# NTV-UIT/MARLLB

Hardware: NVIDIA B200
Metric: agent-steps/sec (higher is better)
Workload: dtype f32

## Files before the change

### marllb_b200/csrc/mlb_features.cuh

```cuda
#pragma once
#include "mlb_common.cuh"

namespace mlb {

#define MLB_WP_MARGIN 5e-5f

template <int EPL, int SIZE, int STRIDE>
__device__ __forceinline__ void bitonic_stage(float (&k)[EPL], float (&p)[EPL], int lane) {
    if constexpr (STRIDE >= EPL) {
        constexpr int LSTRIDE = STRIDE / EPL;
        const bool keep_min = (((lane * EPL) & SIZE) == 0) == ((lane & LSTRIDE) == 0);
#pragma unroll
        for (int r = 0; r < EPL; r++) {
            const float ok = __shfl_xor_sync(MLB_FULL, k[r], LSTRIDE);
            const float op = __shfl_xor_sync(MLB_FULL, p[r], LSTRIDE);
            const float nk = keep_min ? fminf(k[r], ok) : fmaxf(k[r], ok);
            p[r] = (nk != k[r]) ? op : p[r];
            k[r] = nk;
        }
    } else {
#pragma unroll
        for (int r = 0; r < EPL; r++) {
            if ((r & STRIDE) == 0) {
                const int r2 = r | STRIDE;
// ... 181 lines not shown
    __syncwarp();
    bool ambiguous;
    int idx = weighted_index_scan_f64(vw, n, tmax, decay, &ambiguous);
    if (ambiguous) idx = weighted_index_f64(vw, n, now, decay);
    return idx;
}

__device__ __forceinline__ float fast_rcp(float x) {
    float y;
    asm("rcp.approx.ftz.f32 %0, %1;" : "=f"(y) : "f"(x));
    return y;
}
__device__ __forceinline__ float fast_sqrt(float x) {
    float y;
    asm("sqrt.approx.ftz.f32 %0, %1;" : "=f"(y) : "f"(x));
    return y;
}

template <int EPL, bool FULL>
__device__ __forceinline__ void features_ranked(const float (&v)[EPL], const float (&t)[EPL],
                                                const int (&rk)[EPL], int n_, float now, double decay,
                                                float log2_decay, const WarpScratch& sc, float (&out)[5]) {
    const int lane = lane_id();
    const int s0 = lane * EPL;
    const int n = FULL ? 32 * EPL : n_;
    float s = 0.f, tmax = -MLB_INF;
#pragma unroll
    for (int r = 0; r < EPL; r++) {
        const bool valid = FULL || s0 + r < n;
        s += valid ? v[r] : 0.f;
        tmax = valid ? fmaxf(tmax, t[r]) : tmax;
    }
    const float nf = (float)n;
    const float mean = warp_sum(s) / nf;
    tmax = f32_from_orderable(__reduce_max_sync(MLB_FULL, f32_orderable(tmax)));
    float s2 = 0.f, svw = 0.f;
#pragma unroll
    for (int r = 0; r < EPL; r++) {
        const bool valid = FULL || s0 + r < n;
        const float d = v[r] - mean;
        s2 += valid ? d * d : 0.f;
        const float w = valid ? fast_exp2(log2_decay * (tmax - t[r])) : 0.f;
        svw += valid ? v[r] * w : 0.f;
        const int pos = valid ? rk[r] : s0 + r;
        sc.vw[pos] = make_float2(v[r], w);
    }
    const float sd = fast_sqrt(warp_sum(s2) / nf);
    svw = warp_sum(svw);
    __syncwarp();
    float cum[EPL];
    float sw = 0.f;
#pragma unroll
    for (int r = 0; r < EPL; r += 2) {
        if constexpr (EPL == 1) {
            sw += sc.vw[s0].y;
            cum[0] = sw;
        } else {
            const float4 q = *reinterpret_cast<const float4*>(sc.vw + s0 + r);
            sw += q.y;
            cum[r] = sw;
            sw += q.w;
            cum[r + 1] = sw;
        }
    }
    const float incl = warp_scan_incl(sw, lane);
    const float W = __shfl_sync(MLB_FULL, incl, 31);
    const float mean_decay = svw * fast_rcp(W);
    const float rel = 0.9f * W - (incl - sw);
    int below = 0;
    float dmin = MLB_INF;
#pragma unroll
    for (int r = 0; r < EPL; r++) {
        const bool valid = FULL || s0 + r < n;
        below += (valid && cum[r] < rel) ? 1 : 0;
        dmin = valid ? fminf(dmin, fabsf(cum[r] - rel)) : dmin;
    }
    int idx = __reduce_add_sync(MLB_FULL, below);
    const uint32_t dmin_bits = __reduce_min_sync(MLB_FULL, __float_as_uint(dmin));
    if (__uint_as_float(dmin_bits) < MLB_WP_MARGIN * W) {
        SlotVals<EPL> tv;
        uint32_t packed = 0;
#pragma unroll
        for (int r = 0; r < EPL; r++) {
            tv.x[r] = t[r];
            packed |= (uint32_t)(rk[r] & 255) << (8 * r);
        }
        idx = weighted_index_exact<EPL>(tv, packed, n, tmax, now, decay, sc.vw);
    }
    idx = idx > n - 1 ? n - 1 : idx;
    const float vidx = (float)(n - 1) * (90.0f / 100.0f);
    const float fl = floorf(vidx);
    int lo = (int)fl, hi = lo + 1;
    if (vidx >= (float)(n - 1)) { lo = n - 1; hi = n - 1; }
    hi = hi > n - 1 ? n - 1 : hi;
    const float gamma = vidx - fl;
    const float a = sc.vw[lo].x, b = sc.vw[hi].x;
    const float p90_decay = sc.vw[idx].x;
    const float diff = __fsub_rn(b, a);
    float p90 = __fadd_rn(a, __fmul_rn(diff, gamma));
    if (gamma >= 0.5f) p90 = __fsub_rn(b, __fmul_rn(diff, __fsub_rn(1.0f, gamma)));
    __syncwarp();
    out[0] = mean;
    out[1] = p90;
    out[2] = sd;
    out[3] = mean_decay;
    out[4] = p90_decay;
}

template <int EPL>
__device__ __forceinline__ void features_sorted_epl(const float* __restrict__ vals, const float* __restrict__ tss,
                                                    uint8_t* __restrict__ ranks, int n, float now, double decay,
                                                    float log2_decay, const WarpScratch& sc, float (&out)[5]) {
    const int lane = lane_id();
    float v[EPL], t[EPL];
    int rk[EPL];
    load_slots<EPL>(vals, lane, v);
    load_slots<EPL>(tss, lane, t);
    ranks_full_sort<EPL>(v, n, rk, sc);
    if (ranks) store_ranks<EPL>(ranks, lane, rk);
    if (n == 32 * EPL)
        features_ranked<EPL, true>(v, t, rk, n, now, decay, log2_decay, sc, out);
    else
        features_ranked<EPL, false>(v, t, rk, n, now, decay, log2_decay, sc, out);
}

__device__ __forceinline__ float half_sum(float v) {
#pragma unroll
    for (int o = 8; o > 0; o >>= 1) v += __shfl_xor_sync(MLB_FULL, v, o, 16);
    return v;
}
__device__ __forceinline__ uint32_t half_reduce_add_u16(uint32_t x, int half) {
    const uint32_t both = __reduce_add_sync(MLB_FULL, half ? (x << 16) : x);
    return half ? (both >> 16) : (both & 0xffffu);
}
__device__ __forceinline__ uint32_t half_reduce_max(uint32_t x, int half) {
    const uint32_t m0 = __reduce_max_sync(MLB_FULL, half ? 0u : x);
    const uint32_t m1 = __reduce_max_sync(MLB_FULL, half ? x : 0u);
    return half ? m1 : m0;
}
__device__ __forceinline__ uint32_t half_reduce_min(uint32_t x, int half) {
    const uint32_t m0 = __reduce_min_sync(MLB_FULL, half ? 0xffffffffu : x);
    const uint32_t m1 = __reduce_min_sync(MLB_FULL, half ? x : 0xffffffffu);
    return half ? m1 : m0;
}

template <typename T>
__device__ __forceinline__ T pick8(const T (&x)[8], int sub) {
    const T a = (sub & 1) ? x[1] : x[0], b = (sub & 1) ? x[3] : x[2];
    const T c = (sub & 1) ? x[5] : x[4], d = (sub & 1) ? x[7] : x[6];
    const T lo = (sub & 2) ? b : a, hi = (sub & 2) ? d : c;
    return (sub & 4) ? hi : lo;
}

__device__ __forceinline__ void rank_replace_one_h16(const float (&v)[8], uint32_t (&rkp)[2], int c, int hl,
                                                     int half) {
    const int sub = c & 7, lc = c >> 3;
    const float x = __shfl_sync(MLB_FULL, pick8(v, sub), lc, 16) + 0.0f;
    const uint32_t wsel = (sub & 4) ? rkp[1] : rkp[0];
    const uint32_t r_old = (__shfl_sync(MLB_FULL, wsel, lc, 16) >> (8 * (sub & 3))) & 255u;
    const uint32_t xb = __float_as_uint(x);
    const float xup = __uint_as_float((xb >> 31) ? xb - 1u : xb + 1u);
    const int dl = c - hl * 8;
    uint32_t bef0 = 0, bef1 = 0;
#pragma unroll
    for (int r = 0; r < 4; r++) {
        bef0 |= v[r] < (r == dl ? x : xup) ? (1u << (8 * r)) : 0u;
        bef1 |= v[r + 4] < (r + 4 == dl ? x : xup) ? (1u << (8 * r)) : 0u;
    }
    const uint32_t r_new = half_reduce_add_u16((uint32_t)(__popc(bef0) + __popc(bef1)), half);
    const uint32_t rep = (r_old + 1u) * 0x01010101u;
    rkp[0] = rkp[0] - ((((rkp[0] | 0x80808080u) - rep) >> 7) & 0x01010101u) + (bef0 ^ 0x01010101u);
    rkp[1] = rkp[1] - ((((rkp[1] | 0x80808080u) - rep) >> 7) & 0x01010101u) + (bef1 ^ 0x01010101u);
    if (hl == lc) {
        const int sh = 8 * (sub & 3);
        if (sub & 4) rkp[1] = (rkp[1] & ~(255u << sh)) | (r_new << sh);
        else rkp[0] = (rkp[0] & ~(255u << sh)) | (r_new << sh);
    }
}

__device__ __forceinline__ bool features_full_h16(const float (&v)[8], const float (&t)[8], const uint32_t (&rkp)[2],
                                                  float log2_decay, float2* vw, int hl, int half,
                                                  float (&out)[5]) {
    const float s = ((v[0] + v[1]) + (v[2] + v[3])) + ((v[4] + v[5]) + (v[6] + v[7]));
    const float tm = fmaxf(fmaxf(fmaxf(t[0], t[1]), fmaxf(t[2], t[3])), fmaxf(fmaxf(t[4], t[5]), fmaxf(t[6], t[7])));
    const float mean = half_sum(s) * (1.0f / 128.0f);
    const float tmax = f32_from_orderable(half_reduce_max(f32_orderable(tm), half));
    float s2 = 0.f, svw = 0.f;
#pragma unroll
    for (int r = 0; r < 8; r++) {
        const float dv = v[r] - mean;
        s2 += dv * dv;
        const float w = fast_exp2(log2_decay * (tmax - t[r]));
        svw += v[r] * w;
        const uint32_t pos = (rkp[r >> 2] >> (8 * (r & 3))) & 255u;
        vw[((pos & 7u) << 4) | (pos >> 3)] = make_float2(v[r], w);
    }
    const float sd = fast_sqrt(half_sum(s2) * (1.0f / 128.0f));
    svw = half_sum(svw);
    __syncwarp();
    float cum[8];
    float sw = 0.f;
#pragma unroll
    for (int r = 0; r < 8; r++) {
        sw += vw[r * 16 + hl].y;
        cum[r] = sw;
    }
    float incl = sw;
#pragma unroll
    for (int o = 1; o < 16; o <<= 1) {
        const float y = __shfl_up_sync(MLB_FULL, incl, o, 16);
        if (hl >= o) incl += y;
    }
    const float W = __shfl_sync(MLB_FULL, incl, 15, 16);
    const float mean_decay = svw * fast_rcp(W);
    const float rel = 0.9f * W - (incl - sw);
    int below = 0;
    float dmin = MLB_INF;
#pragma unroll
    for (int r = 0; r < 8; r++) {
        below += cum[r] < rel ? 1 : 0;
        dmin = fminf(dmin, fabsf(cum[r] - rel));
    }
    int idx = (int)half_reduce_add_u16((uint32_t)below, half);
    const uint32_t dmin_bits = half_reduce_min(__float_as_uint(dmin), half);
    const bool ok = !(__uint_as_float(dmin_bits) < MLB_WP_MARGIN * W);
    idx = idx > 127 ? 127 : idx;
    const float vidx = 127.0f * (90.0f / 100.0f);
    const float fl = floorf(vidx);
    const int lo = (int)fl, hi = lo + 1;
    const float gamma = vidx - fl;
    const float a = vw[((lo & 7) << 4) | (lo >> 3)].x, b = vw[((hi & 7) << 4) | (hi >> 3)].x;
    const float p90_decay = vw[((idx & 7) << 4) | (idx >> 3)].x;
    const float diff = __fsub_rn(b, a);
    float p90 = __fadd_rn(a, __fmul_rn(diff, gamma));
    if (gamma >= 0.5f) p90 = __fsub_rn(b, __fmul_rn(diff, __fsub_rn(1.0f, gamma)));
    __syncwarp();
    out[0] = mean;
    out[1] = p90;
    out[2] = sd;
    out[3] = mean_decay;
    out[4] = p90_decay;
    return ok;
}

__device__ __forceinline__ void rank_update_h16(const float (&v)[8], uint32_t (&rkp)[2], uint32_t list, int nchg,
                                                int n_old, int hl, int half) {
    const int s0 = hl * 8;
    uint32_t pm0 = 0, pm1 = 0;
#pragma unroll
    for (int r = 0; r < 4; r++) {
        pm0 |= (s0 + r < n_old) ? (1u << (8 * r)) : 0u;
        pm1 |= (s0 + 4 + r < n_old) ? (1u << (8 * r)) : 0u;
    }
#pragma unroll 1
    for (int k = 0; k < 3; k++) {
        const int c = (list >> (7 * k)) & 127;
        const bool rem = k < nchg && c < n_old;
        if (!__any_sync(MLB_FULL, rem)) continue;
        const int sub = c & 7, lc = c >> 3;
        const uint32_t wsel = (sub & 4) ? rkp[1] : rkp[0];
        const uint32_t r_old = (__shfl_sync(MLB_FULL, wsel, lc, 16) >> (8 * (sub & 3))) & 255u;
        const uint32_t rep = ((r_old & 127u) + 1u) * 0x01010101u;
        const uint32_t g0 = ((((rkp[0] | 0x80808080u) - rep) >> 7) & pm0);
        const uint32_t g1 = ((((rkp[1] | 0x80808080u) - rep) >> 7) & pm1);
        if (rem) {
            rkp[0] -= g0;
            rkp[1] -= g1;
            if (hl == lc) {
                if (sub & 4) pm1 &= ~(1u << (8 * (sub & 3))); else pm0 &= ~(1u << (8 * (sub & 3)));
            }
        }
    }
#pragma unroll 1
    for (int k = 0; k < 3; k++) {
        const bool ins = k < nchg;
        if (!__any_sync(MLB_FULL, ins)) break;
        const int c = (list >> (7 * k)) & 127;
        const int sub = c & 7, lc = c >> 3;
        const float x = __shfl_sync(MLB_FULL, pick8(v, sub), lc, 16) + 0.0f;
        const uint32_t xb = __float_as_uint(x);
        const float xup = __uint_as_float((xb >> 31) ? xb - 1u : xb + 1u);
        uint32_t bef0 = 0, bef1 = 0;
#pragma unroll
        for (int r = 0; r < 4; r++) {
            bef0 |= v[r] < xup ? (1u << (8 * r)) : 0u;
            bef1 |= v[r + 4] < xup ? (1u << (8 * r)) : 0u;
        }
        const uint32_t r_new = half_reduce_add_u16((uint32_t)(__popc(bef0 & pm0) + __popc(bef1 & pm1)), half);
        if (ins) {
            rkp[0] += ~bef0 & pm0;
            rkp[1] += ~bef1 & pm1;
            if (hl == lc) {
                const int sh = 8 * (sub & 3);
                if (sub & 4) { rkp[1] = (rkp[1] & ~(255u << sh)) | (r_new << sh); pm1 |= 1u << sh; }
                else { rkp[0] = (rkp[0] & ~(255u << sh)) | (r_new << sh); pm0 |= 1u << sh; }
            }
        }
    }
}

__device__ __forceinline__ bool features_any_h16(const float (&v)[8], const float (&t)[8], const uint32_t (&rkp)[2],
                                                 int n, float log2_decay, float2* vw, int hl, int half,
                                                 float (&out)[5]) {
    const int s0 = hl * 8;
    float s = 0.f, tm = -MLB_INF;
#pragma unroll
    for (int r = 0; r < 8; r++) {
        const bool valid = s0 + r < n;
        s += valid ? v[r] : 0.f;
        tm = valid ? fmaxf(tm, t[r]) : tm;
    }
    const float nf = (float)n;
    const float mean = half_sum(s) / nf;
    const float tmax = f32_from_orderable(half_reduce_max(f32_orderable(tm), half));
    float s2 = 0.f, svw = 0.f;
#pragma unroll
    for (int r = 0; r < 8; r++) {
        const bool valid = s0 + r < n;
        const float dv = v[r] - mean;
        s2 += valid ? dv * dv : 0.f;
        const float w = valid ? fast_exp2(log2_decay * (tmax - t[r])) : 0.f;
        svw += valid ? v[r] * w : 0.f;
        const uint32_t pos = valid ? ((rkp[r >> 2] >> (8 * (r & 3))) & 127u) : (uint32_t)(s0 + r);
        vw[((pos & 7u) << 4) | (pos >> 3)] = make_float2(v[r], w);
    }
    const float sd = fast_sqrt(half_sum(s2) / nf);
    svw = half_sum(svw);
    __syncwarp();
    float cum[8];
    float sw = 0.f;
#pragma unroll
    for (int r = 0; r < 8; r++) {
        sw += vw[r * 16 + hl].y;
        cum[r] = sw;
    }
    float incl = sw;
#pragma unroll
    for (int o = 1; o < 16; o <<= 1) {
        const float y = __shfl_up_sync(MLB_FULL, incl, o, 16);
        if (hl >= o) incl += y;
    }
    const float W = __shfl_sync(MLB_FULL, incl, 15, 16);
    const float mean_decay = svw * fast_rcp(W);
    const float rel = 0.9f * W - (incl - sw);
    int below = 0;
    float dmin = MLB_INF;
#pragma unroll
    for (int r = 0; r < 8; r++) {
        const bool valid = s0 + r < n;
        below += (valid && cum[r] < rel) ? 1 : 0;
        dmin = valid ? fminf(dmin, fabsf(cum[r] - rel)) : dmin;
    }
    int idx = (int)half_reduce_add_u16((uint32_t)below, half);
    const uint32_t dmin_bits = half_reduce_min(__float_as_uint(dmin), half);
    const bool ok = !(__uint_as_float(dmin_bits) < MLB_WP_MARGIN * W);
    idx = idx > n - 1 ? n - 1 : idx;
    const float vidx = (float)(n - 1) * (90.0f / 100.0f);
    const float fl = floorf(vidx);
    int lo = (int)fl, hi = lo + 1;
    if (vidx >= (float)(n - 1)) { lo = n - 1; hi = n - 1; }
    hi = hi > n - 1 ? n - 1 : hi;
    const float gamma = vidx - fl;
    const float a = vw[((lo & 7) << 4) | (lo >> 3)].x, b = vw[((hi & 7) << 4) | (hi >> 3)].x;
    const float p90_decay = vw[((idx & 7) << 4) | (idx >> 3)].x;
    const float diff = __fsub_rn(b, a);
    float p90 = __fadd_rn(a, __fmul_rn(diff, gamma));
    if (gamma >= 0.5f) p90 = __fsub_rn(b, __fmul_rn(diff, __fsub_rn(1.0f, gamma)));
    __syncwarp();
    out[0] = mean;
    out[1] = p90;
    out[2] = sd;
    out[3] = mean_decay;
    out[4] = p90_decay;
    return ok;
}

__device__ __forceinline__ float feature_of_lane(const float (&f)[5], int lane) {
    float mine = f[0];
#pragma unroll
    for (int q = 1; q < 5; q++) mine = lane == q ? f[q] : mine;
    return mine;
}

static __device__ __noinline__ float warp_features_sorted(const float* __restrict__ vals, const float* __restrict__ tss,
                                                          uint8_t* __restrict__ ranks, int n, float now, double decay,
                                                          float log2_decay, float2* scratch) {
    const WarpScratch sc{scratch};
    float f[5];
    if (n <= 0) {
#pragma unroll
        for (int q = 0; q < 5; q++) f[q] = 0.f;
    } else if (n <= 32) {
        features_sorted_epl<1>(vals, tss, ranks, n, now, decay, log2_decay, sc, f);
    } else if (n <= 64) {
        features_sorted_epl<2>(vals, tss, ranks, n, now, decay, log2_decay, sc, f);
    } else {
        features_sorted_epl<4>(vals, tss, ranks, n, now, decay, log2_decay, sc, f);
    }
    return feature_of_lane(f, lane_id());
}

static __device__ __noinline__ float warp_features_ranked_exact(const float* __restrict__ vals, const float* __restrict__ tss,
                                                                const uint8_t* __restrict__ ranks, int n, float now,
                                                                double decay, float log2_decay, float2* scratch) {
    const WarpScratch sc{scratch};
    const int lane = lane_id();
    float v[4], t[4], f[5];
    int rk[4];
    load_slots<4>(vals, lane, v);
    load_slots<4>(tss, lane, t);
    load_ranks<4>(ranks, lane, rk);
    features_ranked<4, false>(v, t, rk, n, now, decay, log2_decay, sc, f);
    return feature_of_lane(f, lane);
}

}
```

### marllb_b200/csrc/mlb_step_kernel.cuh

```cuda
#pragma once
#include "mlb_common.cuh"
#include "mlb_env.cuh"
#include "mlb_features.cuh"
#include "../../include/marllb_b200.h"

namespace mlb {

enum : int {
    F_NON = 0,
    F_LASTFIN,
    F_HEAD,
    F_ACT,
    F_CNT0, F_CNT1,
    F_CUR0, F_CUR1,
    F_CHG0, F_CHG1,
    F_SPEED,
    NF
};

__device__ __forceinline__ uint32_t chg_count(uint32_t w) { return (w >> 21) & 7u; }
__device__ __forceinline__ uint32_t chg_nold(uint32_t w) { return w >> 24; }

__host__ __device__ inline size_t event_warp_smem_bytes(int SP, bool alias) {
    return (size_t)NF * SP * 4 + (alias ? (size_t)SP * (8 + 4 + 8 + 4) : 0);
// ... 304 lines not shown
            for (int m = 0; m < 2; m++) {
                const size_t c = ((size_t)e * 2 + m) * S + seed0 + j;
                const uint32_t cnt = d.res_count[c];
                sm[(F_CNT0 + m) * SP + j] = cnt;
                sm[(F_CUR0 + m) * SP + j] = d.res_cursor[c];
                sm[(F_CHG0 + m) * SP + j] = (cnt < (uint32_t)d.K ? cnt : (uint32_t)d.K) << 24;
            }
        }
    });
    __syncwarp();
    if (kAlias) {
        for (int j = lane; j < Sa; j += 32) {
            const uint32_t act = sm[F_ACT * SP + j];
            a_w[j] = d.action_kind == MLB_ACTION_CONTINUOUS_F32 ? __uint_as_float(act) : d.dw[act];
        }
        __syncwarp();
        if (lane == 0) alias_build(a_prob, a_alias, a_alias + SP, a_w, Sa);
        __syncwarp();
    }

    const int64_t aoff = d.arr_off[ea];
    const int an = d.arr_n[ea];
    int cur = d.arr_cur[ea];
    for (;;) {
        const int idx = cur + lane;
        const float at = idx < an ? __ldcs(d.arr_time + aoff + idx) : MLB_INF;
        const unsigned bal = __ballot_sync(MLB_FULL, at < t1);
        const int nv = (bal == MLB_FULL) ? 32 : (__ffs(~bal) - 1);
        const bool last = nv < 32;
        const float awk = idx < an ? __ldcs(d.arr_work + aoff + idx) : 0.f;
        int abk = 0;
        float au = 0.f;
        if ((kAlias || kPo2) && lane < nv) {
            abk = __ldcs(d.arr_bucket + aoff + idx);
            if (kAlias) au = __ldcs(d.arr_u + aoff + idx);
        }
        const int iters = nv + (last ? 1 : 0);
        for (int i = 0; i < iters; i++) {
            const bool real = i < nv;
            const float ash = __shfl_sync(MLB_FULL, at, i & 31);
            const float wk = __shfl_sync(MLB_FULL, awk, i & 31);
            const float a = real ? ash : t1;
            static_for<R>([&](auto rc) {
                constexpr int r = decltype(rc)::value;
                if (hf[r] < a) {
                    const int j = lane + 32 * r;
                    uint32_t h = sm[F_HEAD * SP + j];
                    int n = (int)sm[F_NON * SP + j];
                    float fin = hf[r], arr = ha[r];
                    do {
                        h = (h + 1 == (uint32_t)Q) ? 0u : h + 1;
                        n -= 1;
                        float2 nx = make_float2(0.f, MLB_INF);
                        if (n > 0) nx = d.ring[g.ring + j * Q + h];
                        res_add<SP, RNG>(d, sm, g, 0, j, __fsub_rn(fin, arr), fin);
                        arr = nx.x;
                        fin = nx.y;
                    } while (fin < a);
                    hf[r] = fin;
                    ha[r] = arr;
                    sm[F_HEAD * SP + j] = h;
                    sm[F_NON * SP + j] = (uint32_t)n;
                    if (kArgmin) sc[r] = server_score<POLICY>(d, n, sm[F_ACT * SP + j]);
                }
            });
            __syncwarp();
            if (!real) break;
            int kstar;
            if (kAlias) {
                const int b = __shfl_sync(MLB_FULL, abk, i);
                const float u = __shfl_sync(MLB_FULL, au, i);
                kstar = ((double)u < a_prob[b]) ? b : a_alias[b];
            } else if (kPo2) {
                const int c0 = __shfl_sync(MLB_FULL, abk, i);
                const int c1 = (c0 + 1 == Sa) ? 0 : c0 + 1;
                const uint32_t s0 = server_score<POLICY>(d, (int)sm[F_NON * SP + c0], sm[F_ACT * SP + c0]);
                const uint32_t s1 = server_score<POLICY>(d, (int)sm[F_NON * SP + c1], sm[F_ACT * SP + c1]);
                kstar = s1 < s0 ? c1 : c0;
            } else {
                uint32_t bkey = sc[0];
                int bj = lane;
                static_for<R>([&](auto rc) {
                    constexpr int r = decltype(rc)::value;
                    if (r > 0 && sc[r] < bkey) { bkey = sc[r]; bj = lane + 32 * r; }
                });
                const uint32_t mkey = __reduce_min_sync(MLB_FULL, bkey);
                kstar = (int)__reduce_min_sync(MLB_FULL, (uint32_t)(bkey == mkey ? bj : 0x7fffffff));
            }
            if (lane == (kstar & 31)) {
                const int k = kstar;
                const int n = (int)sm[F_NON * SP + k];
                if (n >= Q) {
                    atomicAdd(d.dropped + sbase + k, 1u);
                } else {
                    const float start = fmaxf(smf[F_LASTFIN * SP + k], a);
                    const float fin = __fadd_rn(start, __fdiv_rn(wk, smf[F_SPEED * SP + k]));
                    uint32_t pos = sm[F_HEAD * SP + k] + (uint32_t)n;
                    if (pos >= (uint32_t)Q) pos -= (uint32_t)Q;
                    d.ring[g.ring + k * Q + pos] = make_float2(a, fin);
                    smf[F_LASTFIN * SP + k] = fin;
                    sm[F_NON * SP + k] = (uint32_t)(n + 1);
                    uint32_t nsc = 0;
                    if (kArgmin) nsc = server_score<POLICY>(d, n + 1, sm[F_ACT * SP + k]);
                    static_for<R>([&](auto rc) {
                        constexpr int r = decltype(rc)::value;
                        if ((k >> 5) == r) {
                            if (n == 0) { hf[r] = fin; ha[r] = a; }
                            sc[r] = nsc;
                        }
                    });
                }
                if (d.record_assign) d.assign[aoff + cur + i] = seed0 + k;
            }
            __syncwarp();
        }
        cur += nv;
        if (last) break;
    }
    if (lane == 0) d.arr_cur[ea] = cur;

    float* obs = d.obs + sbase * MLB_OBS_COLS;
    static_for<R>([&](auto rc) {
        constexpr int r = decltype(rc)::value;
        const int j = lane + 32 * r;
        if (j < Sa) {
            const size_t gi = sbase + j;
            const int n = (int)sm[F_NON * SP + j];
            uint32_t pos = sm[F_HEAD * SP + j];
            d.n_on[gi] = n;
            d.last_fin[gi] = smf[F_LASTFIN * SP + j];
            d.head[gi] = pos;
            obs[j * MLB_OBS_COLS] = (float)n;
            float arr = ha[r];
            for (int q = 0; q < n; q++) {
                pos = (pos + 1 == (uint32_t)Q) ? 0u : pos + 1;
                float nx = 0.f;
                if (q + 1 < n) nx = d.ring[g.ring + j * Q + pos].x;
                res_add<SP, RNG>(d, sm, g, 1, j, __fsub_rn(t1, arr), t1);
                arr = nx;
            }
#pragma unroll
            for (int m = 0; m < 2; m++) {
                const size_t c = ((size_t)e * 2 + m) * S + seed0 + j;
                d.res_count[c] = sm[(F_CNT0 + m) * SP + j];
                d.res_cursor[c] = sm[(F_CUR0 + m) * SP + j];
                d.res_chg[c] = sm[(F_CHG0 + m) * SP + j];
            }
        }
    });
}

#define MLB_STAGE_BYTES 1152
__host__ __device__ inline size_t pair_warp_smem_bytes(int SP) {
    return (size_t)2 * SP * 8 + 2 * MLB_SCRATCH_BYTES + 2 * MLB_STAGE_BYTES;
}

template <int R, int CLS>
__global__ void __launch_bounds__(128, 8)
pair_kernel(const __grid_constant__ DevState d) {
    extern __shared__ __align__(16) unsigned char smem_raw[];
    constexpr int SP = 32 * R;
    const int lane = threadIdx.x & 31;
    const int warp = threadIdx.x >> 5;
    const int A = d.A, Sa = d.Sa, S = d.S;
    const int wpe = d.pair_wpe;
    const int ea = d.e0 * A + (wpe == 1 ? blockIdx.x * (blockDim.x >> 5) + warp : (int)blockIdx.x);
    const int sub = wpe == 1 ? 0 : warp;
    if (ea >= d.e1 * A) return;
    const int e = ea / A;
    const int agent = ea - e * A;
    unsigned char* wbase = smem_raw + (size_t)warp * pair_warp_smem_bytes(SP);
    uint2* dlist = reinterpret_cast<uint2*>(wbase);
    float2* const vw = reinterpret_cast<float2*>(wbase + (size_t)2 * SP * 8);
    unsigned char* stage = wbase + (size_t)2 * SP * 8 + 2 * MLB_SCRATCH_BYTES;
    const size_t sbase = (size_t)e * S + (size_t)agent * Sa;
    const int seed0 = agent * Sa;

    int nfast = 0;
#pragma unroll
    for (int r = 0; r < R; r++) {
        const int j = lane + 32 * r;
#pragma unroll
        for (int m = 0; m < 2; m++) {
            uint32_t chg = 0, cnt = 0;
            if (j < Sa) {
                const size_t c = ((size_t)e * 2 + m) * S + seed0 + j;
                chg = __ldg(d.res_chg + c);
                cnt = __ldg(d.res_count + c);
            }
            const uint32_t nchg = chg_count(chg);
            const uint32_t n = cnt < (uint32_t)d.K ? cnt : (uint32_t)d.K;
            const bool one = nchg == 1 && chg_nold(chg) == 128 && n == 128;
            const bool redo = chg_nold(chg) == 255u;
            const bool inc = !redo && chg_nold(chg) > 0 && nchg >= 1 && nchg <= 3;
            const bool fast = j < Sa && (CLS == 0 ? one : (inc && !one));
            const unsigned bal = __ballot_sync(MLB_FULL, fast);
            if (fast) dlist[nfast + __popc(bal & ((1u << lane) - 1u))] = make_uint2(chg, (uint32_t)(j * 2 + m) | (n << 9));
            nfast += __popc(bal);
        }
    }
    __syncwarp();
    if (nfast == 0) return;
    const float4* const val4 = reinterpret_cast<const float4*>(d.res_val);
    const float4* const ts4 = reinterpret_cast<const float4*>(d.res_ts);
    uint32_t* const rank4 = reinterpret_cast<uint32_t*>(d.res_rank);
    uint32_t off0 = (uint32_t)(sbase * 2 * 32) + (uint32_t)lane;
    uint32_t obs0 = (uint32_t)(sbase * MLB_OBS_COLS) + 1u;
    uint32_t chg0 = (uint32_t)((size_t)e * 2 * S + seed0);
    asm volatile("" : "+r"(off0), "+r"(obs0), "+r"(chg0));
    const uint32_t stage_s = (uint32_t)__cvta_generic_to_shared(stage) + lane * 16;
    const int half = lane >> 4, hl = lane & 15;
    float2* const vw_half = vw + half * 128;
    auto stage_in = [&](uint32_t id, int slot) {
        const uint32_t off = off0 + id * 32u;
        const uint32_t dst = stage_s + (uint32_t)slot * MLB_STAGE_BYTES;
        cp_async16(dst, val4 + off);
        cp_async16(dst + 512, ts4 + off);
        cp_async4(dst + 1024 - lane * 12, rank4 + off);
    };
    const int i0 = 2 * sub, di = 2 * wpe;
    if (i0 >= nfast) return;
    stage_in(dlist[i0].y & 511u, 0);
    if (i0 + 1 < nfast) stage_in(dlist[i0 + 1].y & 511u, 1);
    cp_async_commit();
#pragma unroll 1
    for (int i = i0; i < nfast; i += di) {
        const bool valid = i + half < nfast;
        const uint2 ent = dlist[valid ? i + half : i];
        const uint32_t id = ent.y & 511u;
        cp_async_wait_all();
        __syncwarp();
        const unsigned char* rec = stage + half * MLB_STAGE_BYTES;
        const float4 v0 = reinterpret_cast<const float4*>(rec)[hl * 2], v1 = reinterpret_cast<const float4*>(rec)[hl * 2 + 1];
        const float4 t0 = reinterpret_cast<const float4*>(rec + 512)[hl * 2], t1q = reinterpret_cast<const float4*>(rec + 512)[hl * 2 + 1];
        const uint2 rq = reinterpret_cast<const uint2*>(rec + 1024)[hl];
        __syncwarp();
        if (i + di < nfast) {
            stage_in(dlist[i + di].y & 511u, 0);
            if (i + di + 1 < nfast) stage_in(dlist[i + di + 1].y & 511u, 1);
            cp_async_commit();
        }
        const float v[8] = {v0.x, v0.y, v0.z, v0.w, v1.x, v1.y, v1.z, v1.w};
        const float t[8] = {t0.x, t0.y, t0.z, t0.w, t1q.x, t1q.y, t1q.z, t1q.w};
        uint32_t rkp[2] = {valid ? rq.x : 0u, valid ? rq.y : 0u};
        float f[5];
        bool ok;
        if (CLS == 0) {
            rank_replace_one_h16(v, rkp, (int)(ent.x & 127u), hl, half);
            if (valid) reinterpret_cast<uint2*>(rank4 + (off0 - lane + id * 32u))[hl] = make_uint2(rkp[0], rkp[1]);
            if (!valid) { rkp[0] = 0u; rkp[1] = 0u; }
            ok = features_full_h16(v, t, rkp, d.log2_decay, vw_half, hl, half, f);
        } else {
            const int n = valid ? (int)((ent.y >> 9) & 255u) : 1;
            rank_update_h16(v, rkp, ent.x, valid ? (int)chg_count(ent.x) : 0, valid ? (int)chg_nold(ent.x) : 1, hl, half);
            if (valid) reinterpret_cast<uint2*>(rank4 + (off0 - lane + id * 32u))[hl] = make_uint2(rkp[0], rkp[1]);
            if (!valid) { rkp[0] = 0u; rkp[1] = 0u; }
            ok = features_any_h16(v, t, rkp, n, d.log2_decay, vw_half, hl, half, f);
        }
        if (valid && hl == 0) {
            if (ok) {
                float* o = d.obs + (obs0 + (id >> 1) * MLB_OBS_COLS + (id & 1u) * 5u);
#pragma unroll
                for (int q = 0; q < 5; q++) o[q] = f[q];
            } else {
                d.res_chg[chg0 + (id & 1u) * (uint32_t)S + (id >> 1)] = (ent.x & 0x00ffffffu) | (255u << 24);
            }
        }
    }
}

template <int R, bool SMALL>
__global__ void __launch_bounds__(SMALL ? 128 : 1024, SMALL ? 12 : 1)
feature_kernel(const __grid_constant__ DevState d) {
    extern __shared__ __align__(16) unsigned char smem_raw[];
    constexpr int SP = 32 * R;
    const int lane = threadIdx.x & 31;
    const int warp = threadIdx.x >> 5;
    const int A = d.A, Sa = d.Sa, S = d.S;
    const int nwarps = blockDim.x >> 5;
    const int epb = nwarps / A;
    const int env_in_blk = warp / A;
    const int agent = warp - env_in_blk * A;
    const int e = d.e0 + blockIdx.x * epb + env_in_blk;
    if (e >= d.e1) return;

    const size_t wbytes = feature_warp_smem_bytes(SP);
    unsigned char* wbase = smem_raw + (size_t)warp * wbytes;
    uint2* dlist = reinterpret_cast<uint2*>(wbase);
    const WarpScratch scratch{reinterpret_cast<float2*>(wbase + (size_t)2 * SP * 8)};
    float* rv = reinterpret_cast<float*>(smem_raw + (size_t)nwarps * wbytes) + (size_t)env_in_blk * 2 * S;
    uint32_t* ra = reinterpret_cast<uint32_t*>(rv + S);

    const int step = d.step[e] + 1;
    const float t1 = __fmul_rn((float)step, d.dt);
    const size_t sbase = (size_t)e * S + (size_t)agent * Sa;
    const int seed0 = agent * Sa;
    float* const res_val = d.res_val + sbase * 2 * d.KP;
    float* const res_ts = d.res_ts + sbase * 2 * d.KP;
    uint8_t* const res_rank = d.res_rank + sbase * 2 * d.KP;
    float* const obs = d.obs + sbase * MLB_OBS_COLS;

    const bool all = d.feature_cache == 0;
    const int KP = d.KP;
    int nd = 0;
#pragma unroll
    for (int r = 0; r < R; r++) {
        const int j = lane + 32 * r;
#pragma unroll
        for (int m = 0; m < 2; m++) {
            uint32_t chg = 0, cnt = 0;
            if (j < Sa) {
                const size_t c = ((size_t)e * 2 + m) * S + seed0 + j;
                chg = __ldg(d.res_chg + c);
                cnt = __ldg(d.res_count + c);
            }
            const uint32_t nchg = chg_count(chg);
            const uint32_t n = cnt < (uint32_t)d.K ? cnt : (uint32_t)d.K;
            const bool redo = chg_nold(chg) == 255u;
            const bool fast = d.use_pair && !redo && chg_nold(chg) > 0 && nchg >= 1 && nchg <= 3;
            const bool take = j < Sa && (all || nchg > 0) && !fast;
            const unsigned bal = __ballot_sync(MLB_FULL, take);
            if (take)
                dlist[nd + __popc(bal & ((1u << lane) - 1u))] =
                    make_uint2(chg, (uint32_t)(j * 2 + m) | (n << 9) | ((redo ? 1u : 0u) << 18));
            nd += __popc(bal);
        }
    }
    __syncwarp();
    float* const warp_obs = obs + 1;
#pragma unroll 1
    for (int i = 0; i < nd; i++) {
        const uint2 ent = dlist[i];
        const uint32_t id = ent.y & 511u;
        const int n = (int)((ent.y >> 9) & 255u);
        const int rid = (int)id * KP;
        float mine;
        if ((ent.y >> 18) & 1u)
            mine = warp_features_ranked_exact(res_val + rid, res_ts + rid, res_rank + rid, n, t1, d.decay,
                                              d.log2_decay, scratch.vw);
        else
            mine = warp_features_sorted(res_val + rid, res_ts + rid, res_rank + rid, n, t1, d.decay,
                                        d.log2_decay, scratch.vw);
        if (lane < 5) warp_obs[(id >> 1) * MLB_OBS_COLS + (id & 1u) * 5u + lane] = mine;
    }
    __syncwarp();

#pragma unroll 1
    for (int j = lane; j < Sa; j += 32) {
        const float* row = obs + j * MLB_OBS_COLS;
        bool active = false;
        float x = 0.f;
#pragma unroll
        for (int c = 0; c < MLB_OBS_COLS; c++) {
            const float o = row[c];
            active |= o > 0.f;
            x = c == d.reward_field ? o : x;
        }
        rv[seed0 + j] = x;
        ra[seed0 + j] = active ? 1u : 0u;
    }
    if (A == 1) {
        __syncwarp();
    } else if (env_in_blk == 0) {
        asm volatile("bar.sync 1, %0;" ::"r"(A * 32) : "memory");
    } else {
        asm volatile("bar.sync 2, %0;" ::"r"(A * 32) : "memory");
    }
    if (agent == 0) {
        const double rw = reward_staged<float>(d.reward_metric, rv, ra, S);
        if (lane == 0) {
            d.reward[e] = rw;
            d.done[e] = step >= d.max_steps ? 1 : 0;
            d.step[e] = step;
        }
    }
}

}
```

Before: 34.80 million.

## Split incremental pair work into full/append/any classes with specialised rank and feature paths

Measured after the change: 35.38 million (median of 6 runs). 1.7% higher.

```diff
diff --git a/marllb_b200/csrc/mlb_features.cuh b/marllb_b200/csrc/mlb_features.cuh
--- a/marllb_b200/csrc/mlb_features.cuh
+++ b/marllb_b200/csrc/mlb_features.cuh
@@ -448,20 +448,22 @@
     return ok;
 }
 
+enum : int { RK_ANY = 0, RK_FULL = 1, RK_APPEND = 2 };
+template <int MODE>
 __device__ __forceinline__ void rank_update_h16(const float (&v)[8], uint32_t (&rkp)[2], uint32_t list, int nchg,
                                                 int n_old, int hl, int half) {
     const int s0 = hl * 8;
-    uint32_t pm0 = 0, pm1 = 0;
-#pragma unroll
-    for (int r = 0; r < 4; r++) {
-        pm0 |= (s0 + r < n_old) ? (1u << (8 * r)) : 0u;
-        pm1 |= (s0 + 4 + r < n_old) ? (1u << (8 * r)) : 0u;
-    }
-#pragma unroll 1
-    for (int k = 0; k < 3; k++) {
+    uint32_t pm0 = 0x01010101u, pm1 = 0x01010101u;
+    if (MODE != RK_FULL) {
+        pm0 = 0; pm1 = 0;
+#pragma unroll
+        for (int r = 0; r < 4; r++) {
+            pm0 |= (s0 + r < n_old) ? (1u << (8 * r)) : 0u;
+            pm1 |= (s0 + 4 + r < n_old) ? (1u << (8 * r)) : 0u;
+        }
+    }
+    auto remove = [&](int k, bool rem) {
         const int c = (list >> (7 * k)) & 127;
-        const bool rem = k < nchg && c < n_old;
-        if (!__any_sync(MLB_FULL, rem)) continue;
         const int sub = c & 7, lc = c >> 3;
         const uint32_t wsel = (sub & 4) ? rkp[1] : rkp[0];
         const uint32_t r_old = (__shfl_sync(MLB_FULL, wsel, lc, 16) >> (8 * (sub & 3))) & 255u;
@@ -475,11 +477,8 @@
                 if (sub & 4) pm1 &= ~(1u << (8 * (sub & 3))); else pm0 &= ~(1u << (8 * (sub & 3)));
             }
         }
-    }
-#pragma unroll 1
-    for (int k = 0; k < 3; k++) {
-        const bool ins = k < nchg;
-        if (!__any_sync(MLB_FULL, ins)) break;
+    };
+    auto insert = [&](int k, bool ins) {
         const int c = (list >> (7 * k)) & 127;
         const int sub = c & 7, lc = c >> 3;
         const float x = __shfl_sync(MLB_FULL, pick8(v, sub), lc, 16) + 0.0f;
@@ -501,17 +500,44 @@
                 else { rkp[0] = (rkp[0] & ~(255u << sh)) | (r_new << sh); pm0 |= 1u << sh; }
             }
         }
-    }
-}
-
+    };
+    if constexpr (MODE == RK_ANY) {
+#pragma unroll 1
+        for (int k = 0; k < 3; k++) {
+            const int c = (list >> (7 * k)) & 127;
+            const bool rem = k < nchg && c < n_old;
+            if (!__any_sync(MLB_FULL, rem)) continue;
+            remove(k, rem);
+        }
+#pragma unroll 1
+        for (int k = 0; k < 3; k++) {
+            const bool ins = k < nchg;
+            if (!__any_sync(MLB_FULL, ins)) break;
+            insert(k, ins);
+        }
+    } else {
+        if constexpr (MODE == RK_FULL) {
+            remove(0, nchg > 0);
+            remove(1, nchg > 1);
+            if (__any_sync(MLB_FULL, nchg > 2)) remove(2, nchg > 2);
+        }
+        insert(0, nchg > 0);
+        if (MODE == RK_FULL || __any_sync(MLB_FULL, nchg > 1)) insert(1, nchg > 1);
+        if (__any_sync(MLB_FULL, nchg > 2)) insert(2, nchg > 2);
+    }
+}
+
+template <int N>
 __device__ __forceinline__ bool features_any_h16(const float (&v)[8], const float (&t)[8], const uint32_t (&rkp)[2],
-                                                 int n, float log2_decay, float2* vw, int hl, int half,
+                                                 int n_, float log2_decay, float2* vw, int hl, int half,
                                                  float (&out)[5]) {
+    static_assert(N == 0 || N == 128, "N: 0 (run-time n) or 128");
     const int s0 = hl * 8;
+    const int n = N ? N : n_;
     float s = 0.f, tm = -MLB_INF;
 #pragma unroll
     for (int r = 0; r < 8; r++) {
-        const bool valid = s0 + r < n;
+        const bool valid = N == 128 || s0 + r < n;
         s += valid ? v[r] : 0.f;
         tm = valid ? fmaxf(tm, t[r]) : tm;
     }
@@ -521,11 +547,13 @@
     float s2 = 0.f, svw = 0.f;
 #pragma unroll
     for (int r = 0; r < 8; r++) {
-        const bool valid = s0 + r < n;
+        const bool valid = N == 128 || s0 + r < n;
         const float dv = v[r] - mean;
-        s2 += valid ? dv * dv : 0.f;
-        const float w = valid ? fast_exp2(log2_decay * (tmax - t[r])) : 0.f;
-        svw += valid ? v[r] * w : 0.f;
+        s2 += valid ? __fmul_rn(dv, dv) : 0.f;
+        float e;
+        asm volatile("ex2.approx.ftz.f32 %0, %1;" : "=f"(e) : "f"(log2_decay * (tmax - t[r])));
+        const float w = valid ? e : 0.f;
+        svw += valid ? __fmul_rn(v[r], w) : 0.f;
         const uint32_t pos = valid ? ((rkp[r >> 2] >> (8 * (r & 3))) & 127u) : (uint32_t)(s0 + r);
         vw[((pos & 7u) << 4) | (pos >> 3)] = make_float2(v[r], w);
     }
@@ -552,7 +580,7 @@
     float dmin = MLB_INF;
 #pragma unroll
     for (int r = 0; r < 8; r++) {
-        const bool valid = s0 + r < n;
+        const bool valid = N == 128 || s0 + r < n;
         below += (valid && cum[r] < rel) ? 1 : 0;
         dmin = valid ? fminf(dmin, fabsf(cum[r] - rel)) : dmin;
     }
diff --git a/marllb_b200/csrc/mlb_step_kernel.cuh b/marllb_b200/csrc/mlb_step_kernel.cuh
--- a/marllb_b200/csrc/mlb_step_kernel.cuh
+++ b/marllb_b200/csrc/mlb_step_kernel.cuh
@@ -480,8 +480,11 @@
 
 #define MLB_STAGE_BYTES 1152
 __host__ __device__ inline size_t pair_warp_smem_bytes(int SP) {
-    return (size_t)2 * SP * 8 + 2 * MLB_SCRATCH_BYTES + 2 * MLB_STAGE_BYTES;
-}
+    return (size_t)(2 * SP + 2) * 8 + 2 * MLB_SCRATCH_BYTES + 2 * MLB_STAGE_BYTES;
+}
+
+enum : uint32_t { PC_ONE = 0, PC_F2 = 0, PC_APPEND = 1, PC_ANY = 2, PC_NONE = 3 };
+#define MLB_PAIR_PAD (1u << 31)
 
 template <int R, int CLS>
 __global__ void __launch_bounds__(128, 8)
@@ -499,12 +502,13 @@
     const int agent = ea - e * A;
     unsigned char* wbase = smem_raw + (size_t)warp * pair_warp_smem_bytes(SP);
     uint2* dlist = reinterpret_cast<uint2*>(wbase);
-    float2* const vw = reinterpret_cast<float2*>(wbase + (size_t)2 * SP * 8);
-    unsigned char* stage = wbase + (size_t)2 * SP * 8 + 2 * MLB_SCRATCH_BYTES;
+    float2* const vw = reinterpret_cast<float2*>(wbase + (size_t)(2 * SP + 2) * 8);
+    unsigned char* stage = wbase + (size_t)(2 * SP + 2) * 8 + 2 * MLB_SCRATCH_BYTES;
     const size_t sbase = (size_t)e * S + (size_t)agent * Sa;
     const int seed0 = agent * Sa;
 
-    int nfast = 0;
+    uint2 cand[2 * R];
+    uint32_t cls_of = 0;
 #pragma unroll
     for (int r = 0; r < R; r++) {
         const int j = lane + 32 * r;
@@ -516,15 +520,41 @@
                 chg = __ldg(d.res_chg + c);
                 cnt = __ldg(d.res_count + c);
             }
-            const uint32_t nchg = chg_count(chg);
+            const uint32_t nchg = chg_count(chg), nold = chg_nold(chg);
             const uint32_t n = cnt < (uint32_t)d.K ? cnt : (uint32_t)d.K;
-            const bool one = nchg == 1 && chg_nold(chg) == 128 && n == 128;
-            const bool redo = chg_nold(chg) == 255u;
-            const bool inc = !redo && chg_nold(chg) > 0 && nchg >= 1 && nchg <= 3;
-            const bool fast = j < Sa && (CLS == 0 ? one : (inc && !one));
-            const unsigned bal = __ballot_sync(MLB_FULL, fast);
-            if (fast) dlist[nfast + __popc(bal & ((1u << lane) - 1u))] = make_uint2(chg, (uint32_t)(j * 2 + m) | (n << 9));
+            const bool one = nchg == 1 && nold == 128 && n == 128;
+            const bool redo = nold == 255u;
+            const bool inc = !redo && nold > 0 && nchg >= 1 && nchg <= 3;
+            uint32_t cls = PC_NONE;
+            if (CLS == 0) {
+                cls = one ? PC_ONE : PC_NONE;
+            } else if (inc && !one) {
+                bool app = nold + nchg == n;
+#pragma unroll
+                for (int k = 0; k < 3; k++) app = app && ((uint32_t)k >= nchg || ((chg >> (7 * k)) & 127u) >= nold);
+                cls = nold == 128 && n == 128 ? PC_F2 : (app ? PC_APPEND : PC_ANY);
+            }
+            if (j >= Sa) cls = PC_NONE;
+            cand[2 * r + m] = make_uint2(chg, (uint32_t)(j * 2 + m) | (n << 9));
+            cls_of |= cls << (2 * (2 * r + m));
+        }
+    }
+    int nfast = 0, end_f2 = 0, end_app = 0;
+#pragma unroll
+    for (uint32_t c = 0; c < (CLS == 0 ? 1u : 3u); c++) {
+#pragma unroll
+        for (int q = 0; q < 2 * R; q++) {
+            const bool take = ((cls_of >> (2 * q)) & 3u) == c;
+            const unsigned bal = __ballot_sync(MLB_FULL, take);
+            if (take) dlist[nfast + __popc(bal & ((1u << lane) - 1u))] = cand[q];
             nfast += __popc(bal);
+        }
+        if (CLS == 1 && c < 2) {
+            if (nfast & 1) {
+                if (lane == 0) dlist[nfast] = make_uint2(0u, MLB_PAIR_PAD);
+                nfast++;
+            }
+            (c == 0 ? end_f2 : end_app) = nfast;
         }
     }
     __syncwarp();
@@ -551,10 +581,10 @@
     stage_in(dlist[i0].y & 511u, 0);
     if (i0 + 1 < nfast) stage_in(dlist[i0 + 1].y & 511u, 1);
     cp_async_commit();
-#pragma unroll 1
-    for (int i = i0; i < nfast; i += di) {
-        const bool valid = i + half < nfast;
-        const uint2 ent = dlist[valid ? i + half : i];
+    auto pair_step = [&](int i, auto kc) {
+        constexpr uint32_t KC = decltype(kc)::value;
+        const uint2 ent = dlist[i + half < nfast ? i + half : i];
+        const bool valid = i + half < nfast && ent.y != MLB_PAIR_PAD;
         const uint32_t id = ent.y & 511u;
         cp_async_wait_all();
         __syncwarp();
@@ -571,6 +601,7 @@
         const float v[8] = {v0.x, v0.y, v0.z, v0.w, v1.x, v1.y, v1.z, v1.w};
         const float t[8] = {t0.x, t0.y, t0.z, t0.w, t1q.x, t1q.y, t1q.z, t1q.w};
         uint32_t rkp[2] = {valid ? rq.x : 0u, valid ? rq.y : 0u};
+        const int nchg = valid ? (int)chg_count(ent.x) : 0;
         float f[5];
         bool ok;
         if (CLS == 0) {
@@ -578,12 +609,18 @@
             if (valid) reinterpret_cast<uint2*>(rank4 + (off0 - lane + id * 32u))[hl] = make_uint2(rkp[0], rkp[1]);
             if (!valid) { rkp[0] = 0u; rkp[1] = 0u; }
             ok = features_full_h16(v, t, rkp, d.log2_decay, vw_half, hl, half, f);
+        } else if (KC == PC_F2) {
+            rank_update_h16<RK_FULL>(v, rkp, ent.x, nchg, 128, hl, half);
+            if (valid) reinterpret_cast<uint2*>(rank4 + (off0 - lane + id * 32u))[hl] = make_uint2(rkp[0], rkp[1]);
+            if (!valid) { rkp[0] = 0u; rkp[1] = 0u; }
+            ok = features_any_h16<128>(v, t, rkp, 128, d.log2_decay, vw_half, hl, half, f);
         } else {
             const int n = valid ? (int)((ent.y >> 9) & 255u) : 1;
-            rank_update_h16(v, rkp, ent.x, valid ? (int)chg_count(ent.x) : 0, valid ? (int)chg_nold(ent.x) : 1, hl, half);
+            const int nold = valid ? (int)chg_nold(ent.x) : 1;
+            rank_update_h16<KC == PC_APPEND ? RK_APPEND : RK_ANY>(v, rkp, ent.x, nchg, nold, hl, half);
             if (valid) reinterpret_cast<uint2*>(rank4 + (off0 - lane + id * 32u))[hl] = make_uint2(rkp[0], rkp[1]);
             if (!valid) { rkp[0] = 0u; rkp[1] = 0u; }
-            ok = features_any_h16(v, t, rkp, n, d.log2_decay, vw_half, hl, half, f);
+            ok = features_any_h16<0>(v, t, rkp, n, d.log2_decay, vw_half, hl, half, f);
         }
         if (valid && hl == 0) {
             if (ok) {
@@ -594,7 +631,16 @@
                 d.res_chg[chg0 + (id & 1u) * (uint32_t)S + (id >> 1)] = (ent.x & 0x00ffffffu) | (255u << 24);
             }
         }
-    }
+    };
+    int i = i0;
+    if (CLS == 1) {
+#pragma unroll 1
+        for (; i < end_f2; i += di) pair_step(i, std::integral_constant<uint32_t, PC_F2>{});
+#pragma unroll 1
+        for (; i < end_app; i += di) pair_step(i, std::integral_constant<uint32_t, PC_APPEND>{});
+    }
+#pragma unroll 1
+    for (; i < nfast; i += di) pair_step(i, std::integral_constant<uint32_t, CLS == 0 ? PC_ONE : PC_ANY>{});
 }
 
 template <int R, bool SMALL>
```

## Handle multi-change full windows and append-only updates with batched rank update

Applied to the files above, without the earlier changes.

New measurement: 34.72 million before, 34.95 million after (median of 6 runs). About the same (+0.7%).

```diff
diff --git a/marllb_b200/csrc/mlb_features.cuh b/marllb_b200/csrc/mlb_features.cuh
--- a/marllb_b200/csrc/mlb_features.cuh
+++ b/marllb_b200/csrc/mlb_features.cuh
@@ -357,29 +357,70 @@
     return (sub & 4) ? hi : lo;
 }
 
-__device__ __forceinline__ void rank_replace_one_h16(const float (&v)[8], uint32_t (&rkp)[2], int c, int hl,
-                                                     int half) {
-    const int sub = c & 7, lc = c >> 3;
-    const float x = __shfl_sync(MLB_FULL, pick8(v, sub), lc, 16) + 0.0f;
-    const uint32_t wsel = (sub & 4) ? rkp[1] : rkp[0];
-    const uint32_t r_old = (__shfl_sync(MLB_FULL, wsel, lc, 16) >> (8 * (sub & 3))) & 255u;
-    const uint32_t xb = __float_as_uint(x);
-    const float xup = __uint_as_float((xb >> 31) ? xb - 1u : xb + 1u);
-    const int dl = c - hl * 8;
-    uint32_t bef0 = 0, bef1 = 0;
-#pragma unroll
-    for (int r = 0; r < 4; r++) {
-        bef0 |= v[r] < (r == dl ? x : xup) ? (1u << (8 * r)) : 0u;
-        bef1 |= v[r + 4] < (r + 4 == dl ? x : xup) ? (1u << (8 * r)) : 0u;
-    }
-    const uint32_t r_new = half_reduce_add_u16((uint32_t)(__popc(bef0) + __popc(bef1)), half);
-    const uint32_t rep = (r_old + 1u) * 0x01010101u;
-    rkp[0] = rkp[0] - ((((rkp[0] | 0x80808080u) - rep) >> 7) & 0x01010101u) + (bef0 ^ 0x01010101u);
-    rkp[1] = rkp[1] - ((((rkp[1] | 0x80808080u) - rep) >> 7) & 0x01010101u) + (bef1 ^ 0x01010101u);
-    if (hl == lc) {
-        const int sh = 8 * (sub & 3);
-        if (sub & 4) rkp[1] = (rkp[1] & ~(255u << sh)) | (r_new << sh);
-        else rkp[0] = (rkp[0] & ~(255u << sh)) | (r_new << sh);
+template <bool FULL, int KMAX>
+__device__ __forceinline__ void rank_update_few_h16(const float (&v)[8], uint32_t (&rkp)[2], uint32_t list, int nc,
+                                                    int n_old, int hl, int half) {
+    const int ncmax = KMAX == 1 ? 1 : (int)__reduce_max_sync(MLB_FULL, (uint32_t)nc);
+    const int s0 = hl * 8;
+    uint32_t cm0 = 0x01010101u, cm1 = 0x01010101u, pm0 = 0x01010101u, pm1 = 0x01010101u;
+    if (!FULL) {
+        cm0 = cm1 = pm0 = pm1 = 0u;
+#pragma unroll
+        for (int r = 0; r < 4; r++) {
+            cm0 |= (s0 + r < n_old + nc) ? (1u << (8 * r)) : 0u;
+            cm1 |= (s0 + 4 + r < n_old + nc) ? (1u << (8 * r)) : 0u;
+            pm0 |= (s0 + r < n_old) ? (1u << (8 * r)) : 0u;
+            pm1 |= (s0 + 4 + r < n_old) ? (1u << (8 * r)) : 0u;
+        }
+    }
+    float x[3];
+    uint32_t cnt[3];
+    uint32_t dec0 = 0, dec1 = 0, inc0 = 0, inc1 = 0;
+#pragma unroll
+    for (int k = 0; k < KMAX; k++) {
+        x[k] = 0.f;
+        cnt[k] = 0u;
+        if (k < ncmax) {
+            const int c = (list >> (7 * k)) & 127;
+            const int sub = c & 7, lc = c >> 3;
+            const uint32_t on = k < nc ? 0x01010101u : 0u;
+            x[k] = __shfl_sync(MLB_FULL, pick8(v, sub), lc, 16) + 0.0f;
+            if (FULL) {
+                const uint32_t wsel = (sub & 4) ? rkp[1] : rkp[0];
+                const uint32_t r_old = (__shfl_sync(MLB_FULL, wsel, lc, 16) >> (8 * (sub & 3))) & 255u;
+                const uint32_t rep = (r_old + 1u) * 0x01010101u;
+                dec0 += (((rkp[0] | 0x80808080u) - rep) >> 7) & on;
+                dec1 += (((rkp[1] | 0x80808080u) - rep) >> 7) & on;
+            }
+            const uint32_t xb = __float_as_uint(x[k]);
+            const float xup = __uint_as_float((xb >> 31) ? xb - 1u : xb + 1u);
+            uint32_t bef0 = 0, bef1 = 0;
+#pragma unroll
+            for (int r = 0; r < 4; r++) {
+                bef0 |= v[r] < xup ? (1u << (8 * r)) : 0u;
+                bef1 |= v[r + 4] < xup ? (1u << (8 * r)) : 0u;
+            }
+            cnt[k] = half_reduce_add_u16((uint32_t)(__popc(bef0 & cm0) + __popc(bef1 & cm1)), half);
+            inc0 += ~bef0 & pm0 & on;
+            inc1 += ~bef1 & pm1 & on;
+        }
+    }
+    rkp[0] = rkp[0] - dec0 + inc0;
+    rkp[1] = rkp[1] - dec1 + inc1;
+#pragma unroll
+    for (int k = 0; k < KMAX; k++) {
+        if (k < ncmax) {
+            const int c = (list >> (7 * k)) & 127;
+            const int sub = c & 7;
+            uint32_t r_new = cnt[k] - 1u;
+#pragma unroll
+            for (int k2 = k + 1; k2 < KMAX; k2++) r_new -= (k2 < nc && x[k2] == x[k]) ? 1u : 0u;
+            if (k < nc && hl == (c >> 3)) {
+                const int sh = 8 * (sub & 3);
+                if (sub & 4) rkp[1] = (rkp[1] & ~(255u << sh)) | (r_new << sh);
+                else rkp[0] = (rkp[0] & ~(255u << sh)) | (r_new << sh);
+            }
+        }
     }
 }
 
diff --git a/marllb_b200/csrc/mlb_step_kernel.cuh b/marllb_b200/csrc/mlb_step_kernel.cuh
--- a/marllb_b200/csrc/mlb_step_kernel.cuh
+++ b/marllb_b200/csrc/mlb_step_kernel.cuh
@@ -487,6 +487,7 @@
 __global__ void __launch_bounds__(128, 8)
 pair_kernel(const __grid_constant__ DevState d) {
     extern __shared__ __align__(16) unsigned char smem_raw[];
+    __shared__ int block_nfast;
     constexpr int SP = 32 * R;
     const int lane = threadIdx.x & 31;
     const int warp = threadIdx.x >> 5;
@@ -498,36 +499,53 @@
     const int e = ea / A;
     const int agent = ea - e * A;
     unsigned char* wbase = smem_raw + (size_t)warp * pair_warp_smem_bytes(SP);
-    uint2* dlist = reinterpret_cast<uint2*>(wbase);
+    const uint2* dlist = reinterpret_cast<const uint2*>(wpe == 1 ? wbase : smem_raw);
     float2* const vw = reinterpret_cast<float2*>(wbase + (size_t)2 * SP * 8);
     unsigned char* stage = wbase + (size_t)2 * SP * 8 + 2 * MLB_SCRATCH_BYTES;
     const size_t sbase = (size_t)e * S + (size_t)agent * Sa;
     const int seed0 = agent * Sa;
 
     int nfast = 0;
-#pragma unroll
-    for (int r = 0; r < R; r++) {
-        const int j = lane + 32 * r;
-#pragma unroll
-        for (int m = 0; m < 2; m++) {
-            uint32_t chg = 0, cnt = 0;
-            if (j < Sa) {
-                const size_t c = ((size_t)e * 2 + m) * S + seed0 + j;
-                chg = __ldg(d.res_chg + c);
-                cnt = __ldg(d.res_count + c);
-            }
-            const uint32_t nchg = chg_count(chg);
-            const uint32_t n = cnt < (uint32_t)d.K ? cnt : (uint32_t)d.K;
-            const bool one = nchg == 1 && chg_nold(chg) == 128 && n == 128;
-            const bool redo = chg_nold(chg) == 255u;
-            const bool inc = !redo && chg_nold(chg) > 0 && nchg >= 1 && nchg <= 3;
-            const bool fast = j < Sa && (CLS == 0 ? one : (inc && !one));
-            const unsigned bal = __ballot_sync(MLB_FULL, fast);
-            if (fast) dlist[nfast + __popc(bal & ((1u << lane) - 1u))] = make_uint2(chg, (uint32_t)(j * 2 + m) | (n << 9));
-            nfast += __popc(bal);
-        }
-    }
-    __syncwarp();
+    if (wpe == 1 || warp == 0) {
+        uint2* const wlist = reinterpret_cast<uint2*>(wbase);
+#pragma unroll
+        for (int pass = 0; pass < 2; pass++) {
+#pragma unroll
+            for (int r = 0; r < R; r++) {
+                const int j = lane + 32 * r;
+#pragma unroll
+                for (int m = 0; m < 2; m++) {
+                    uint32_t chg = 0, cnt = 0;
+                    if (j < Sa) {
+                        const size_t c = ((size_t)e * 2 + m) * S + seed0 + j;
+                        chg = __ldcg(d.res_chg + c);
+                        cnt = __ldg(d.res_count + c);
+                    }
+                    const uint32_t nchg = chg_count(chg), nold = chg_nold(chg);
+                    const uint32_t n = cnt < (uint32_t)d.K ? cnt : (uint32_t)d.K;
+                    const bool inc = nold != 255u && nold > 0 && nchg >= 1 && nchg <= 3;
+                    const bool full = nold == 128u;
+                    bool app = true;
+#pragma unroll
+                    for (int k = 0; k < 3; k++) app &= (uint32_t)k >= nchg || ((chg >> (7 * k)) & 127u) >= nold;
+                    const bool first = CLS == 0 ? nchg == 1 : app;
+                    const bool take = j < Sa && inc && (CLS == 0) == full && (pass == 0) == first;
+                    const unsigned bal = __ballot_sync(MLB_FULL, take);
+                    if (take)
+                        wlist[nfast + __popc(bal & ((1u << lane) - 1u))] =
+                            make_uint2(chg, (uint32_t)(j * 2 + m) | (n << 9) | ((first ? 1u : 0u) << 17));
+                    nfast += __popc(bal);
+                }
+            }
+        }
+    }
+    if (wpe != 1) {
+        if (threadIdx.x == 0) block_nfast = nfast;
+        __syncthreads();
+        nfast = block_nfast;
+    } else {
+        __syncwarp();
+    }
     if (nfast == 0) return;
     const float4* const val4 = reinterpret_cast<const float4*>(d.res_val);
     const float4* const ts4 = reinterpret_cast<const float4*>(d.res_ts);
@@ -573,14 +591,23 @@
         uint32_t rkp[2] = {valid ? rq.x : 0u, valid ? rq.y : 0u};
         float f[5];
         bool ok;
+        const int nc = valid ? (int)chg_count(ent.x) : 0;
+        const bool first_pair = __all_sync(MLB_FULL, !valid || ((ent.y >> 17) & 1u));
         if (CLS == 0) {
-            rank_replace_one_h16(v, rkp, (int)(ent.x & 127u), hl, half);
+            if (first_pair)
+                rank_update_few_h16<true, 1>(v, rkp, ent.x, nc, 128, hl, half);
+            else
+                rank_update_few_h16<true, 3>(v, rkp, ent.x, nc, 128, hl, half);
             if (valid) reinterpret_cast<uint2*>(rank4 + (off0 - lane + id * 32u))[hl] = make_uint2(rkp[0], rkp[1]);
             if (!valid) { rkp[0] = 0u; rkp[1] = 0u; }
             ok = features_full_h16(v, t, rkp, d.log2_decay, vw_half, hl, half, f);
         } else {
             const int n = valid ? (int)((ent.y >> 9) & 255u) : 1;
-            rank_update_h16(v, rkp, ent.x, valid ? (int)chg_count(ent.x) : 0, valid ? (int)chg_nold(ent.x) : 1, hl, half);
+            const int n_old = valid ? (int)chg_nold(ent.x) : 1;
+            if (first_pair)
+                rank_update_few_h16<false, 3>(v, rkp, ent.x, nc, n_old, hl, half);
+            else
+                rank_update_h16(v, rkp, ent.x, nc, n_old, hl, half);
             if (valid) reinterpret_cast<uint2*>(rank4 + (off0 - lane + id * 32u))[hl] = make_uint2(rkp[0], rkp[1]);
             if (!valid) { rkp[0] = 0u; rkp[1] = 0u; }
             ok = features_any_h16(v, t, rkp, n, d.log2_decay, vw_half, hl, half, f);
```
